# ShivangNagta/CS201_SAH-BVH_Ray_Tracer

Hardware: AMD Instinct MI355X
Metric: Mrays/s at 1080p, 10k spheres; 1/2/4/8 GPU + CPU baseline (higher is better)
Workload: dtype f32

## Files before the change

cs201_sah-bvh_ray_tracer_amd/abi.py:

```python
import ctypes as C

import numpy as np

VEC3 = ("<f4", (3,))

SPHERE = np.dtype([("center", *VEC3), ("radius", "<f4"), ("color", "u1", (4,))])
RAY = np.dtype([("origin", *VEC3), ("direction", *VEC3)])
AABB = np.dtype([("min", *VEC3), ("max", *VEC3)])
HIT = np.dtype([("t", "<f4"), ("point", *VEC3), ("normal", *VEC3),
                ("hit", "<i4"), ("sphere", "<i4"), ("pad", "<i4")])
NODE = np.dtype([("bmin", *VEC3), ("bmax", *VEC3), ("sphere", "<i4"), ("skip", "<u4")])
CAMERA = np.dtype([("position", *VEC3), ("forward", *VEC3), ("right", *VEC3), ("up", *VEC3),
                   ("yaw", "<f4"), ("pitch", "<f4"), ("fov", "<f4"), ("move", "<i4")])

NODE_EMPTY = 0x80000000
SKIP_MASK = 0x7FFFFFFF

GEO = np.dtype(("<f4", (4,)))
DNODE = np.dtype([("bmin", *VEC3), ("bmax", *VEC3), ("sphere", "<i4"), ("skip", "<u4"),
                  ("geo", "<f4", (4,)), ("pad", "<u4", (4,))])
PNODE = np.dtype([("c0", "<f4", (6,)), ("c1", "<f4", (6,)), ("ref0", "<u4"), ("ref1", "<u4"),
                  ("flat", "<u4"), ("end", "<u4")])
HSLOT = np.dtype([("box", "<u4", (3,)), ("ref", "<u4")])
HNODE = np.dtype([("slot", HSLOT, (4,))])
# ... 190 lines not shown
    ("mirt_accum_download", I, [P, P, C.c_size_t]),
    ("mirt_ctx_share_accum", I, [P, P]),
    ("mirt_ctx_share_scene", I, [P, P]),
    ("mirt_ctx_scene_id", C.c_uint64, [P]),
    ("mirt_trace_rays", I, [P, P, I, I, I, C.c_uint64, C.c_uint32, P]),
    ("mirt_trace_rays_at", I, [P, P, I, I, I, C.c_uint64, C.c_uint32, C.c_uint32, P]),
    ("mirt_camera_rays_uv", I, [P, P, I, I, P, I, P]),
    ("mirt_bvh_overlay", I, [P, P, I, I, I, P]),
    ("mirt_intersect_rays", I, [P, P, I, I, P]),
    ("mirt_any_hit_rays", I, [P, P, I, I, P]),
    ("mirt_sphere_pairs", I, [P, P, P, I, P]),
    ("mirt_aabb_pairs", I, [P, P, P, I, P]),
    ("mirt_hemisphere_probe", I, [P, P, P, P, P, I, P, P]),
    ("mirt_coop_geometry", I, [I, C.c_uint64, P, P, P, P]),
    ("mirt_pixel_rows", I, [I, I, I, I, I, I, P, C.c_int64, P]),
    ("mirt_exact_t_pairs", I, [C.c_int64, P, P, P, P, P, P, P, P]),
    ("mirt_sqrt_form_sweep", I, [P, P, P]),
    ("mirt_box_form_pairs", I, [P, P, P, P, I, I, P]),
    ("mirt_sphere_form_pairs", I, [P, P, P, P, I, I, P]),
    ("mirt_camera_rays", I, [P, P, P, P]),
    ("mirt_count_frame", I, [P, P, P, P]),
    ("mirt_wave_stats", I, [P, P, P, P, I]),
    ("mirt_ctx_stream", P, [P]),
    ("mirt_last_kernel_ms", C.c_float, [P]),
    ("mirt_last_phase_ms", I, [P, C.POINTER(C.c_float)]),
    ("mirt_phase_log", I, [P, C.POINTER(C.c_float), I]),
    ("mirt_bounce_stats", I, [P, P, P, P, I]),
    ("mirt_set_option", I, [P, I, I]),
    ("mirt_get_option", I, [P, I]),
    ("mirt_primary_cache_stats_get", I, [P, P]),
    ("mirt_primary_cache_read", I, [P, P, P, C.c_size_t]),
    ("mirt_primary_cache_write", I, [P, P, P, C.c_size_t]),
    ("mirt_dropin_init", I, [I, I, I]),
    ("mirt_dropin_release", None, []),
# ... 31 lines not shown

OPT_TRAVERSAL, OPT_FAST_SLAB, OPT_BLOCK_WAVES, OPT_DEFER, OPT_BOUNCE_THRESHOLD, OPT_PRUNE, OPT_ORDERED = (
    1, 2, 3, 4, 5, 6, 7)
OPT_BOUNCE_BLOCKS, OPT_QUAD_DRAIN, OPT_LEAF_BATCH, OPT_QUAD_BATCH, OPT_ZERO_COPY = 9, 11, 14, 15, 17
OPT_QUEUE_ORDER, OPT_DEBUG_STALL_MS = 18, 19
OPT_CONFIRM_ONCE, OPT_DEBUG_FAIL_CONFIRM = 21, 22
OPT_BUILD_FINISH = 23
OPT_PRIMARY_CACHE = 24
PCACHE_BYPASS, PCACHE_FILL, PCACHE_HIT = 0, 1, 2
PCACHE_KIND = {PCACHE_BYPASS: "bypass", PCACHE_FILL: "fill", PCACHE_HIT: "hit"}
PCACHE_REASON = {0: "", 1: "EMPTY", 2: "SCENE", 3: "CAMERA", 4: "GEOMETRY", 5: "OFF", 6: "SCHEDULE", 7: "JITTER",
                 8: "PLANES"}
BOUNCE_STATS_WORDS = 23
TRAV_TILE, TRAV_WAVEFRONT = 0, 5
BOX_FORM_SLAB, BOX_FORM_SLAB_BOX, BOX_FORM_CONS, BOX_FORM_CONS_BOUNCE, BOX_FORM_CONS_CAMERA = 0, 1, 2, 3, 4
MULTI_COPY, MULTI_HOST_DIRECT, MULTI_QUEUE_AHEAD = 1, 2, 4
MULTI_FULL_GRID = 1
MULTI_OPT_TIMEOUT_MS, MULTI_OPT_EMULATE_WORLD, MULTI_OPT_EMULATE_RANK, MULTI_OPT_DIRECT_COPY = 256, 257, 258, 259
MULTI_OPT_COPY_STREAM = 260
MULTI_OPT_GATHER_SELF, MULTI_OPT_LEAD_SKIP = 261, 262
```

cs201_sah-bvh_ray_tracer_amd/csrc/coop.h:

```cpp
#pragma once
#include <cstdint>

#include "rng.h"
#include "shard.h"

namespace mirt {

MIRT_HD uint32_t coop_group_shift(uint32_t np)
{
    const uint32_t ceil_log2 = np <= 1u ? 0u : 32u - (uint32_t)__builtin_clz(np - 1u);
    return 6u - ceil_log2;
}
MIRT_HD uint32_t coop_lane_rank(uint32_t lane, uint32_t shift) { return lane >> shift; }
MIRT_HD uint32_t coop_lane_try(uint32_t lane, uint32_t shift) { return lane & ((1u << shift) - 1u); }

MIRT_HD int coop_first_accept(uint64_t accepted, uint32_t rank, uint32_t shift)
{
    uint64_t bits = accepted >> ((rank << shift) & 63u);
    if (shift < 6u) bits &= (1ull << (1u << shift)) - 1ull;
    return bits ? __builtin_ctzll(bits) : -1;
}

struct MagicDiv {
    uint32_t mul, shift;
// ... 17 lines not shown
};
inline RowMagic row_magic_make(int width, int shard_rows, int row_block)
{
    return RowMagic{magic_div_make((uint32_t)width), magic_div_make((uint32_t)shard_rows),
                    magic_div_make((uint32_t)row_block)};
}

MIRT_HD int magic_row_to_y(const RowMagic& m, int r, int samples, int shard_rows, int row_block, int shard,
                           int num_shards, int lead_skip)
{
    if (samples > 1) r -= (int)magic_div((uint32_t)r, (uint32_t)shard_rows, m.shard_rows) * shard_rows;
    const int blk = (int)magic_div((uint32_t)r, (uint32_t)row_block, m.row_block);
    return shard_block(shard, blk, num_shards, lead_skip) * row_block + (r - blk * row_block);
}

}
```

cs201_sah-bvh_ray_tracer_amd/csrc/coop_host.cpp:

```cpp
#include "coop.h"
#include "internal.h"

using namespace mirt;

extern "C" int mirt_coop_geometry(int num_pending, uint64_t accepted, int32_t* group, int32_t* lane_rank,
                                  int32_t* lane_try, int32_t* first_accept)
{
    if (num_pending < 1 || num_pending > 64 || !group || !lane_rank || !lane_try || !first_accept) {
        set_error("mirt_coop_geometry: invalid arguments");
        return MIRT_E_INVALID;
    }
    const uint32_t shift = coop_group_shift((uint32_t)num_pending);
    *group = (int32_t)(1u << shift);
    for (uint32_t i = 0; i < 64; i++) {
        lane_rank[i] = (int32_t)coop_lane_rank(i, shift);
        lane_try[i] = (int32_t)coop_lane_try(i, shift);
    }
    for (uint32_t r = 0; r < (uint32_t)num_pending; r++) first_accept[r] = coop_first_accept(accepted, r, shift);
    return MIRT_OK;
}

extern "C" int mirt_pixel_rows(int width, int shard_rows, int samples, int row_block, int shard, int num_shards,
                               const uint32_t* pixels, int64_t n, int32_t* out)
{
// ... 1 lines not shown
        shard >= num_shards || n < 0 || (n > 0 && (!pixels || !out))) {
        set_error("mirt_pixel_rows: invalid arguments");
        return MIRT_E_INVALID;
    }
    const RowMagic m = row_magic_make(width, shard_rows, row_block);
    for (int64_t i = 0; i < n; i++) {
        const uint32_t p = pixels[i];
        const uint32_t r = magic_div(p, (uint32_t)width, m.width);
        out[4 * i] = (int32_t)r;
        out[4 * i + 1] = (int32_t)(p - r * (uint32_t)width);
        out[4 * i + 2] = magic_row_to_y(m, (int)r, samples, shard_rows, row_block, shard, num_shards, 0);
        out[4 * i + 3] = (int32_t)magic_div(r, (uint32_t)shard_rows, m.shard_rows);
    }
    return MIRT_OK;
}
```

cs201_sah-bvh_ray_tracer_amd/csrc/render.hip:

```cpp
#include <hip/hip_runtime.h>

#include <cmath>
#include <cstdint>
#include <algorithm>
#include <map>
#include <mutex>
#include <cstring>
#include <new>
#include <type_traits>
#include <vector>

#include "coop.h"
#include "internal.h"
#include "shard.h"
#include "trace.h"

using namespace mirt;

namespace {

struct FrameConst {
    float px, py, pz;
    float fx, fy, fz;
    float hx, hy, hz;
// ... 399 lines not shown
        return;
    }
    if (pm) {
        const int leader = __builtin_ctzll(pm);
        uint32_t base = 0;
        if (lane == leader) base = atomicAdd(&qctl[0], (uint32_t)__popcll(pm));
        base = __builtin_amdgcn_readlane(base, leader);
        if (push) queue[base + lanes_below(pm)] = rec;
    }
}

constexpr bool kBoundedSlab = true;
__device__ __forceinline__ SlabRay bounce_slab_ray(const DevScene& sc, const Ray& ray)
{
    SlabRay s = slab_ray(ray);
    s.generic = s.generic ||
                !(sc.o_bound > 0.0f && fmaxf(fabsf(ray.ox), fmaxf(fabsf(ray.oy), fabsf(ray.oz))) <= sc.o_bound);
    return s;
}

__host__ __device__ inline bool origin_within_4c(float o_bound, float o_inf)
{
    return o_bound > 0.0f && o_inf <= 4.0f * o_bound;
}

template <int WALK>
struct BounceWalk;
template <>
struct BounceWalk<0> {
    DfsWalk w;
    __device__ void start(const DevScene& sc) { w = DfsWalk{0u, sc.num_nodes}; }
    __device__ void stop() { w = DfsWalk{kPNone, 0u}; }
// ... 6 lines not shown
        if (w.cur >= w.end) w.cur = kPNone;
    }
};
template <int WALK>
struct WideBounceWalk {
    WideWalk w;
    lds_uint4* hc = nullptr;
    uint32_t hc_n = 0;
    __device__ void start(const DevScene& sc) { w = wide_walk_start(sc, true); }
    __device__ void stop() { w = WideWalk{kPNone, 0u, 0u}; }
    __device__ bool walking() const { return wide_walking(w); }
    template <bool FAST, bool GD = false, bool DEFER = false>
    __device__ void step(const DevScene& sc, const SlabRay& sr, const SphRay& sp, Prune& pr, uint32_t* stk,
                         float& bt, int& bs, Counters& cnt, GateDiag* gd = nullptr, int* lvl = nullptr)
    {
        wide_lane_step<FAST, false, WALK == 4, kBoundedSlab && WALK != 4, GD, DEFER>(sc, sr, sp, pr, w, stk, bt, bs,
                                                                                     cnt, hc, hc_n, gd, lvl);
    }
};
template <>
struct BounceWalk<2> : WideBounceWalk<2> {};
template <>
struct BounceWalk<4> : WideBounceWalk<4> {};


inline size_t bounce_lds_bytes(int depth) { return sizeof(uint32_t) * 256 * (size_t)std::max(depth - 1, 1); }

__device__ __forceinline__ uint64_t chain_key(const FrameConst& f, uint32_t pixel)
{
    const int r = (int)magic_div(pixel, (uint32_t)f.width, f.magic.width), x = (int)(pixel - (uint32_t)r * (uint32_t)f.width);
    return pixel_key(f.seed, (uint32_t)(shard_row_to_y(f, r) * f.width + x), row_sample(f, r));
}

__device__ __forceinline__ bool shade_level(const DevScene& sc, const FrameConst& f, Ray& ray, float best_t,
                                            int best_s, int& level, uint32_t& k, uint64_t key, uint32_t* cs,
                                            int cstride, uint32_t base0, uint32_t pixel, uint32_t* __restrict__ out,
                                            float* __restrict__ acc, bool store)
{
    uint32_t tail = 255u << 24;
    int stored = level - 1;
    if (best_s < 0) {
// ... 49 lines not shown
    for (;;) {
        while (solo_step<FAST, kWideStack * 64, BND>(sc, sr, sp, pr, w, wst, best_t, best_s, hc, hc_n, lane)) {
        }
        if (!shade_level(sc, f, ray, best_t, best_s, level, k, chain_key(f, pixel), cs, kWideStride, base0, pixel, out,
                         acc, lane == 0))
            return;
        sr = bounce_slab_ray(sc, ray);
        sp = sph_ray(ray);
        w = SoloWalk{lane < 4 ? sc.wide_root : kPNone, 0u, 0u};
        best_t = INFINITY;
        best_s = -1;
        pr = prune_off();
    }
}

#define MIRT_BOUNCE_ATTR __attribute__((amdgpu_waves_per_eu(MIRT_BOUNCE_WAVES)))
template <bool FAST, int WALK, bool DIAG = false>
__global__ __launch_bounds__(256) MIRT_BOUNCE_ATTR void bounce_kernel(DevScene sc, FrameConst f, uint32_t* __restrict__ out,
                                                     float* __restrict__ acc, const BounceRec* __restrict__ queue,
                                                     uint32_t* __restrict__ qctl, int threshold, int quad_drain,
                                                     int lvl_mode, int fail_n,
                                                     uint64_t* __restrict__ diag = nullptr)
{
    uint64_t dg_it = 0, dg_lanes = 0, dg_it_x = 0, dg_lanes_x = 0, dg_tx = 0, dg_qit = 0, dg_tq = 0;
    const uint64_t dg_t0 = DIAG ? __builtin_amdgcn_s_memrealtime() : 0;
    uint32_t dg_steps = 0, dg_chain = 0, dg_walk_max = 0, dg_chain_max = 0;
    uint64_t dg_seg = 0, dg_fb = 0, dg_it_gate = 0, dg_it_t = 0, dg_it_box = 0;
    uint32_t dg_conf = 0, dg_conf_fail = 0, dg_fb_exact = 0;
    GateDiag gd{0, 0, 0, 0, 0, false, false, false};
    constexpr bool LANE4 = WALK == 2 || WALK == 4;
// ... 1 lines not shown
    constexpr int cstride = 256;
    extern __shared__ uint32_t cstack[];
    __shared__ uint32_t wstack[LANE4 ? kWideStack * kWideStride : 1];
    __shared__ uint32_t qsrc[LANE4 ? 4 * 16 : 1];
    __shared__ uint4 hcache[LANE4 ? 4 * kHCache : 1];
    uint32_t hc_n = 0;
    if constexpr (LANE4) {
        hc_n = min((uint32_t)kHCache, sc.num_hnodes);
        const uint4* src = (const uint4*)sc.hnodes;
        for (uint32_t i = threadIdx.x; i < 4 * hc_n; i += blockDim.x) hcache[i] = src[i];
        __syncthreads();
    }
    uint32_t tid4 = threadIdx.x << 2;
    if (DEFER) asm volatile("" : "+v"(tid4));
    const uint32_t tid = DEFER ? tid4 >> 2 : threadIdx.x;
    uint32_t* cs = DEFER ? (uint32_t*)((char*)cstack + tid4) : cstack + threadIdx.x;
    uint32_t* stk = DEFER ? (uint32_t*)((char*)wstack + tid4) : wstack + (LANE4 ? threadIdx.x : 0);
    Counters cnt{0, 0, 0, 0, 0};
    const uint32_t n = __builtin_amdgcn_readfirstlane(qctl[0]);
    uint32_t seg = blockIdx.x % kQSeg, segs_left = kQSeg;
    bool has = false, exhausted = false;
    Ray ray{0, 0, 0, 0, 0, 0};
    SlabRay sr = bounce_slab_ray(sc, ray);
    SphRay sp = sph_ray(ray);
    Prune pr = prune_off();
    BounceWalk<WALK> w;
    if constexpr (LANE4) {
        w.hc = (lds_uint4*)hcache;
        w.hc_n = hc_n;
    }
    w.stop();
    uint32_t pixel = 0, k = 0, base0 = 0;
    int level = 0, best_s = -1;
    float best_t = INFINITY;
    for (;;) {
        const uint64_t need = __ballot(!has);
        while (need && !exhausted) {
            const int leader = __builtin_ctzll(need);
            const uint32_t lo = (uint32_t)((uint64_t)n * seg / kQSeg);
            const uint32_t sz = (uint32_t)((uint64_t)n * (seg + 1) / kQSeg) - lo;
            uint32_t b = 0;
            if ((tid & 63) == leader) b = atomicAdd(&qctl[kQLine * (1 + seg)], (uint32_t)__popcll(need));
            b = __builtin_amdgcn_readlane(b, leader);
            if (b + (uint32_t)__popcll(need) >= sz) {
                seg = seg + 1 == kQSeg ? 0 : seg + 1;
                if (--segs_left == 0) exhausted = true;
            }
            if (!has) {
                const uint32_t lane0 = tid & 63;
                const uint32_t idx = b + (uint32_t)__popcll(need & ((1ull << lane0) - 1));
                if (idx < sz) {
                    const BounceRec rec = queue[lo + idx];
                    ray = Ray{rec.ox, rec.oy, rec.oz, rec.dx, rec.dy, rec.dz};
                    sr = bounce_slab_ray(sc, ray);
                    sp = sph_ray(ray);
                    pixel = rec.pixel;
                    k = rec.k;
                    base0 = rec.base0;
                    level = DEFER ? 1 | lvl_mode : 1;
                    w.start(sc);
                    best_t = INFINITY;
                    best_s = -1;
                    pr = prune_off();
                    has = true;
                }
            }
            if (b < sz) break;
        }
        if (!__ballot(has)) break;
        if (DIAG && exhausted && !dg_tx) dg_tx = __builtin_amdgcn_s_memrealtime();
        auto to_drain = [&]() {
            uint32_t busy = (uint32_t)__popcll(__ballot(has));
            asm volatile("" : "+s"(busy));
// ... 34 lines not shown
                dg_it_box += __ballot(gd.st_box) ? 1u : 0u;
            } else if constexpr (DEFER) {
                if (has && w.walking())
                    w.template step<FAST, false, true>(sc, sr, sp, pr, stk, best_t, best_s, cnt, nullptr, &level);
            } else {
                if (has && w.walking()) w.template step<FAST>(sc, sr, sp, pr, stk, best_t, best_s, cnt);
            }
        }
        if constexpr (DEFER) {
            const bool handover = to_drain();
            if (has && (handover || !w.walking()) && !(level & kExactWalk) && best_s >= 0) {
                best_s = confirm_leaf(sc, sr, best_s);
                if (fail_n) {
                    uint32_t fn = (uint32_t)fail_n;
                    asm volatile("" : "+s"(fn));
                    if (pixel % fn == 0) best_s = -1;
                }
                if (DIAG) {
                    dg_conf++;
                    dg_conf_fail += best_s < 0 ? 1u : 0u;
                }
                if (best_s < 0) {
                    level |= kExactWalk;
                    w.start(sc);
                    best_t = INFINITY;
                    pr = prune_off();
                }
            }
            if (handover) break;
        }
        bool go = false;
        float nn[3] = {0.0f, 0.0f, 0.0f};
        uint64_t key = 0;
        if constexpr (WALK == 4) {
            if (has && !w.walking()) {
                go = shade_level(sc, f, ray, best_t, best_s, level, k, chain_key(f, pixel), cs, cstride, base0, pixel,
                                 out, acc, true);
                has = go;
            }
        } else if (has && !w.walking()) {
            if (DEFER) level &= ~kExactWalk;
            if (DIAG) {
                dg_walk_max = max(dg_walk_max, dg_steps);
                dg_chain += dg_steps;
                dg_steps = 0;
            }
            uint32_t tail = 255u << 24;
            int stored = level - 1;
            if (best_s < 0) {
                tail = sky_rgba(ray.dy);
            } else {
                cs[(level - 1) * cstride] = sc.color[best_s];
                stored = level;
                if (level + 1 < f.depth) {
                    float p[3];
                    hit_point_normal(ray, best_t, sc.geo[best_s], p, nn);
                    ray.ox = p[0];
                    ray.oy = p[1];
                    ray.oz = p[2];
                    key = chain_key(f, pixel);
                    level++;
                    go = true;
                }
            }
            if (!go) {
                uint32_t c = tail;
                for (int l = stored - 1; l >= 0; l--) c = blend_rgba(cs[l * cstride], c);
                store_pixel(f, out, acc, pixel, blend_rgba(base0, c));
                has = false;
                if (DIAG) {
                    dg_chain_max = max(dg_chain_max, dg_chain);
                    dg_chain = 0;
                }
            }
        }
        if (WALK != 4 && __ballot(go)) hemisphere_wave(key, k, nn, go, ray.dx, ray.dy, ray.dz, tid & 63);
        if (go) {
            sr = bounce_slab_ray(sc, ray);
            sp = sph_ray(ray);
            w.start(sc);
            best_t = INFINITY;
            best_s = -1;
            pr = prune_off();
            if (DEFER) level |= lvl_mode;
        }
    }
    if constexpr (DEFER) level &= ~kExactWalk;
    if constexpr (LANE4) {
        const uint64_t busy = __ballot(has);
        if (busy) {
            const uint32_t lane = tid & 63, wv = tid >> 6;
            if (has) qsrc[wv * 16 + lanes_below(busy)] = lane;
            __builtin_amdgcn_fence(__ATOMIC_RELEASE, "wavefront");
            __builtin_amdgcn_wave_barrier();
            __builtin_amdgcn_fence(__ATOMIC_ACQUIRE, "wavefront");
            const uint32_t q = lane >> 2;
            const bool qhas = q < (uint32_t)__popcll(busy);
            const uint32_t src = qsrc[wv * 16 + (qhas ? q : 0)];
            auto pull = [&](uint32_t v) { return (uint32_t)__builtin_amdgcn_ds_bpermute((int)(src << 2), (int)v); };
            auto pullf = [&](float v) { return __uint_as_float(pull(__float_as_uint(v))); };
            ray = Ray{pullf(ray.ox), pullf(ray.oy), pullf(ray.oz), pullf(ray.dx), pullf(ray.dy), pullf(ray.dz)};
            pixel = pull(pixel);
            k = pull(k);
            level = (int)pull((uint32_t)level);
            base0 = pull(base0);
            best_t = pullf(best_t);
            best_s = (int)pull((uint32_t)best_s);
            pr = Prune{pullf(pr.m), pullf(pr.lim)};
            const WideWalk& lw = w.w;
            QuadWalk qw{pull(lw.cur), pull(lw.end), pull(lw.top)};
            has = qhas;
            if (!qhas) qw.cur = kPNone;
            sr = bounce_slab_ray(sc, ray);
            sp = sph_ray(ray);
            uint32_t* qstk = wstack + (tid & ~63u) + src;
            uint32_t* qcs = cstack + (tid & ~63u) + src;
            if (DIAG) dg_tq = __builtin_amdgcn_s_memrealtime();
            while (__ballot(has)) {
                if (DIAG) dg_qit++;
                if (!DIAG) {
                    const uint64_t rays = __ballot(has && (lane & 3) == 0);
                    if (__popcll(rays) == 1) {
                        solo_chain<FAST, kBoundedSlab && WALK != 4>(sc, f, __builtin_ctzll(rays), ray, best_t, best_s, pr,
                                                                    qw, level, k, pixel,
                                         base0, src, wstack + (tid & ~63u), cstack + (tid & ~63u),
                                         out, acc, (lds_uint4*)hcache, hc_n, lane);
                        break;
                    }
                }
                if (has && qw.cur != kPNone)
                    quad_step<FAST, kWideStride, kWideStack, kBoundedSlab && WALK != 4>(sc, sr, sp, pr, qw, qstk, best_t,
                                                                                        best_s,
                                                             (lds_uint4*)hcache, hc_n, lane);
                if (has && qw.cur == kPNone) {
                    if (shade_level(sc, f, ray, best_t, best_s, level, k, chain_key(f, pixel), qcs, kWideStride, base0, pixel, out,
                                    acc, (lane & 3) == 0)) {
                        sr = bounce_slab_ray(sc, ray);
                        sp = sph_ray(ray);
                        qw = QuadWalk{sc.wide_root, 0u, 0u};
                        best_t = INFINITY;
// ... 301 lines not shown
        nd.g = make_float4(0.0f, 0.0f, 0.0f, 0.0f);
        pass = slab<true>(sr, pr, nd);
        break;
    }
    case MIRT_BOX_FORM_SLAB_BOX:
        pass = slab_box<true>(sr, pr, b.min.x, b.min.y, b.min.z, b.max.x, b.max.y, b.max.z, near);
        break;
    case MIRT_BOX_FORM_CONS:
        pass = slab_cons<false>(sr, pr, b.min.x, b.min.y, b.min.z, b.max.x, b.max.y, b.max.z, near);
        break;
    case MIRT_BOX_FORM_CONS_BOUNCE:
        sr = bounce_slab_ray(sc, ray);
        pass = slab_cons<true>(sr, pr, b.min.x, b.min.y, b.min.z, b.max.x, b.max.y, b.max.z, near);
        break;
    default:
        sr.generic = sr.generic ||
                     !origin_within_4c(sc.o_bound, fmaxf(fabsf(ray.ox), fmaxf(fabsf(ray.oy), fabsf(ray.oz))));
        pass = slab_cons<true>(sr, pr, b.min.x, b.min.y, b.min.z, b.max.x, b.max.y, b.max.z, near);
        break;
    }
    out[i] = pass ? 1 : 0;
}

template <int MODE>
__global__ void sphere_form_pairs_kernel(const mirt_ray* __restrict__ rays, const mirt_sphere* __restrict__ sph,
                                         const float* __restrict__ best, int n, uint32_t* __restrict__ out)
{
    const int i = blockIdx.x * blockDim.x + threadIdx.x;
    if (i >= n) return;
    const mirt_ray rr = rays[i];
    const Ray ray{rr.origin.x, rr.origin.y, rr.origin.z, rr.direction.x, rr.direction.y, rr.direction.z};
    const float4 g = make_float4(sph[i].center.x, sph[i].center.y, sph[i].center.z, sph[i].radius);
    if constexpr (MODE == 3) {
        bool f64 = false;
        (void)sphere_t<true>(sph_ray(ray), g, best[i], &f64);
        out[i] = f64 ? 1u : 0u;
// ... 1840 lines not shown
    if (n == 0) return MIRT_OK;
    const size_t rb = sizeof(mirt_ray) * (size_t)n, bb = sizeof(mirt_aabb) * (size_t)n, fb = 4 * (size_t)n;
    int rc = ensure(&c->d_in, &c->in_cap, rb + bb + fb + 16);
    if (!rc) rc = ensure(&c->d_res, &c->res_cap, 4 * (size_t)n);
    if (rc) return rc;
    char* din = (char*)c->d_in;
    HIP_TRY(hipMemcpyAsync(din, rays, rb, hipMemcpyHostToDevice, c->stream));
    HIP_TRY(hipMemcpyAsync(din + rb, boxes, bb, hipMemcpyHostToDevice, c->stream));
    HIP_TRY(hipMemcpyAsync(din + rb + bb, best, fb, hipMemcpyHostToDevice, c->stream));
    box_form_pairs_kernel<<<(n + 255) / 256, 256, 0, c->stream>>>(dev_scene(c), (const mirt_ray*)din,
                                                                 (const mirt_aabb*)(din + rb),
                                                                 (const float*)(din + rb + bb), n, form,
                                                                 (int32_t*)c->d_res);
    HIP_TRY(hipGetLastError());
    HIP_TRY(hipMemcpyAsync(out, c->d_res, 4 * (size_t)n, hipMemcpyDeviceToHost, c->stream));
    HIP_TRY(hipStreamSynchronize(c->stream));
    return MIRT_OK;
}

int mirt_sphere_form_pairs(mirt_ctx* c, const mirt_ray* rays, const mirt_sphere* spheres, const float* best, int n,
                           int fast, uint32_t* out)
{
    if (!ctx_ok(c, false, "mirt_sphere_form_pairs")) return MIRT_E_INVALID;
    if (n < 0 || fast < 0 || fast > 3 || (n > 0 && (!rays || !spheres || !best || !out))) {
        set_error("mirt_sphere_form_pairs: invalid arguments");
        return MIRT_E_INVALID;
    }
    if (n == 0) return MIRT_OK;
    const size_t rb = sizeof(mirt_ray) * (size_t)n, sb = sizeof(mirt_sphere) * (size_t)n, fb = 4 * (size_t)n;
    int rc = ensure(&c->d_in, &c->in_cap, rb + sb + fb + 16);
// ... 255 lines not shown
```

cs201_sah-bvh_ray_tracer_amd/csrc/trace.h:

```cpp
#pragma once
#include <hip/hip_runtime.h>

#include <cstdint>

#include "../../include/mirt.h"
#include "coop.h"
#include "exact_t.h"
#include "layout.h"
#include "rng.h"

namespace mirt {

constexpr float kEps = 0.000001f;
constexpr int kMaxDepth = 8;

struct DevScene {
    const DNode* nodes;
    const mirt_node* nodes32;
    const float4* geo;
    const uint32_t* color;
    uint32_t num_nodes;
    int num_spheres;
    int prune;
    float r_max;
// ... 93 lines not shown
        x = y = z = 0.0f;
    }
}

__device__ __forceinline__ float dot3(float ax, float ay, float az, float bx, float by, float bz)
{
    float s = ax * bx;
    s = s + ay * by;
    return s + az * bz;
}

struct SlabRay {
    float ox, oy, oz, dx, dy, dz;
    float ix, iy, iz;
    bool zx, zy, zz;
    bool generic;
};

__device__ __forceinline__ SlabRay slab_ray(const Ray& r)
{
    SlabRay s;
    s.ox = r.ox;
    s.oy = r.oy;
    s.oz = r.oz;
    s.dx = r.dx;
    s.dy = r.dy;
    s.dz = r.dz;
    s.zx = r.dx == 0.0f;
    s.zy = r.dy == 0.0f;
    s.zz = r.dz == 0.0f;
    const float tiny = 0x1p-40f;
    s.generic = !(fabsf(r.dx) >= tiny && fabsf(r.dy) >= tiny && fabsf(r.dz) >= tiny);
    s.ix = 1.0f / r.dx;
    s.iy = 1.0f / r.dy;
    s.iz = 1.0f / r.dz;
    return s;
}

__device__ __forceinline__ bool slab_test(const SlabRay& r, float x0, float y0, float z0, float x1, float y1,
                                          float z1)
{
    float tx1 = -INFINITY, tx2 = INFINITY, ty1 = -INFINITY, ty2 = INFINITY, tz1 = -INFINITY, tz2 = INFINITY;
    if (!r.zx) {
        tx1 = (x0 - r.ox) / r.dx;
        tx2 = (x1 - r.ox) / r.dx;
    }
    if (!r.zy) {
        ty1 = (y0 - r.oy) / r.dy;
        ty2 = (y1 - r.oy) / r.dy;
    }
// ... 510 lines not shown

__device__ __forceinline__ void cx(float& ka, uint32_t& ra, float& kb, uint32_t& rb)
{
    const bool sw = kb < ka;
    const float k = sw ? kb : ka;
    const uint32_t r = sw ? rb : ra;
    kb = sw ? ka : kb;
    rb = sw ? ra : rb;
    ka = k;
    ra = r;
}

__device__ __forceinline__ float h_lo(uint32_t v) { return (float)__builtin_bit_cast(_Float16, (uint16_t)(v & 0xffffu)); }
__device__ __forceinline__ float h_hi(uint32_t v) { return (float)__builtin_bit_cast(_Float16, (uint16_t)(v >> 16)); }

struct GateDiag {
    uint32_t gates, gates_t, gates_box, lanes_t, lanes_box;
    bool st_gate, st_t, st_box;
    __device__ __forceinline__ void gate(bool et, bool eb)
    {
        const uint64_t act = __ballot(true);
        const bool lead =
            __builtin_amdgcn_mbcnt_hi((uint32_t)(act >> 32), __builtin_amdgcn_mbcnt_lo((uint32_t)act, 0u)) == 0;
        const bool any_t = __ballot(et) != 0, any_box = __ballot(eb) != 0;
        gates += lead ? 1u : 0u;
        gates_t += (lead && any_t) ? 1u : 0u;
        gates_box += (lead && any_box) ? 1u : 0u;
        lanes_t += et ? 1u : 0u;
        lanes_box += eb ? 1u : 0u;
        st_gate = true;
// ... 77 lines not shown
{
    const float t = sphere_t<true>(sp, g, best_t);
    if (t > 0.0f) {
        const float4* lp = (const float4*)(sc.leaf_box + (ref & ~kPLeaf));
        const float4 l0 = lp[0], l1 = lp[1];
        const int si = __float_as_int(l1.z);
        float e;
        if ((t < best_t || si > best_s) && slab_box<true>(sr, pr, l0.x, l0.y, l0.z, l0.w, l1.x, l1.y, e)) {
            best_t = t;
            best_s = si;
            if (sc.prune) prune_update(pr, sc, sr.ox, sr.oy, sr.oz, sp.a4(), t);
        }
    }
}

template <bool FAST, bool COUNT, bool BATCH = false, bool BND = false, bool GD = false, bool DEFER = false>
__device__ __forceinline__ void wide_lane_step(const DevScene& sc, const SlabRay& sr, const SphRay& sp, Prune& pr,
                                               WideWalk& w, uint32_t* stk, float& best_t, int& best_s, Counters& cnt,
                                               lds_uint4* hc = nullptr, uint32_t hc_n = 0, GateDiag* gd = nullptr,
                                               int* lvl = nullptr)
{
    static_assert(!DEFER || (FAST && !COUNT && !BATCH), "the deferred gates are the timed lane loop's");
    if (COUNT) cnt.steps++;
    if (w.end) {
        lane_step<FAST, COUNT, true>(sc, sr, sp, pr, w.cur, best_t, best_s, cnt);
        if (w.cur >= w.end) {
            w.end = 0;
            wide_walk_pop(w, stk);
        }
        return;
    }
// ... 3 lines not shown
    {
        uint4 s0, s1, s2, s3;
        if (w.cur < hc_n) {
            lds_uint4* p = hc + 4 * w.cur;
            s0 = lds_load(p);
            s1 = lds_load(p + 1);
            s2 = lds_load(p + 2);
            s3 = lds_load(p + 3);
        } else {
            const uint4* p = (const uint4*)(sc.hnodes + w.cur);
            s0 = p[0];
            s1 = p[1];
            s2 = p[2];
            s3 = p[3];
        }
        auto test = [&](const uint4& q, float& e) {
            if (COUNT && q.w != kPNone) cnt.nodes++;
            const bool pass =
                slab_cons<BND>(sr, pr, h_lo(q.x), h_lo(q.y), h_lo(q.z), h_hi(q.x), h_hi(q.y), h_hi(q.z), e);
            return pass & (q.w != kPNone);
        };
        h0 = test(s0, e0);
        h1 = test(s1, e1);
        h2 = test(s2, e2);
        h3 = test(s3, e3);
        q3 = make_uint4(s0.w, s1.w, s2.w, s3.w);
    }
    uint32_t lm = (uint32_t)(h0 && (q3.x & kPLeaf)) | (uint32_t)(h1 && (q3.y & kPLeaf)) << 1 |
                  (uint32_t)(h2 && (q3.z & kPLeaf)) << 2 | (uint32_t)(h3 && (q3.w & kPLeaf)) << 3;
    h0 = h0 && !(lm & 1);
    h1 = h1 && !(lm & 2);
    h2 = h2 && !(lm & 4);
    h3 = h3 && !(lm & 8);
    const uint32_t n = (uint32_t)h0 + (uint32_t)h1 + (uint32_t)h2 + (uint32_t)h3;
// ... 648 lines not shown
```

cs201_sah-bvh_ray_tracer_amd/renderer.py:

```python
import ctypes as C
import os

import numpy as np

from . import abi
from .lib import MirtError, check, load

ptr = abi.ptr


class RandState:

    def __init__(self, seed=1):
        self.st = abi.RandState()
        load().mirt_srand(C.byref(self.st), seed)

    def rand(self):
        return load().mirt_rand(C.byref(self.st))


def create_random_spheres(n, seed=1, state=None):
    st = state or RandState(seed)
    out = np.zeros(n, abi.SPHERE)
    check(load().mirt_scene_random(C.byref(st.st), ptr(out), n), "mirt_scene_random")
# ... 569 lines not shown
        boxes = np.ascontiguousarray(boxes, abi.AABB)
        out = np.zeros(len(rays), np.int32)
        check(self.L.mirt_aabb_pairs(self.h, ptr(rays), ptr(boxes), len(rays), ptr(out)), "mirt_aabb_pairs")
        return out

    def box_form_pairs(self, rays, boxes, best, form):
        rays = np.ascontiguousarray(rays, abi.RAY)
        boxes = np.ascontiguousarray(boxes, abi.AABB)
        best = np.ascontiguousarray(best, np.float32)
        assert len(boxes) == len(rays) and len(best) == len(rays)
        out = np.zeros(len(rays), np.int32)
        check(self.L.mirt_box_form_pairs(self.h, ptr(rays), ptr(boxes), ptr(best), len(rays), form, ptr(out)),
              "mirt_box_form_pairs")
        return out

    def sphere_form_pairs(self, rays, spheres, best, fast=True):
        rays = np.ascontiguousarray(rays, abi.RAY)
        spheres = np.ascontiguousarray(spheres, abi.SPHERE)
        best = np.ascontiguousarray(best, np.float32)
        assert len(spheres) == len(rays) and len(best) == len(rays)
        out = np.zeros(len(rays), np.uint32)
        check(self.L.mirt_sphere_form_pairs(self.h, ptr(rays), ptr(spheres), ptr(best), len(rays), int(fast),
                                            ptr(out)), "mirt_sphere_form_pairs")
        return out.view(np.float32)

    def sqrt_form_sweep(self):
        bad, first = C.c_uint64(), C.c_uint32()
        check(self.L.mirt_sqrt_form_sweep(self.h, C.byref(bad), C.byref(first)), "mirt_sqrt_form_sweep")
        return bad.value, first.value

# ... 190 lines not shown
```

include/mirt.h:

```cpp
#ifndef MIRT_H
#define MIRT_H

#include <stddef.h>
#include <stdint.h>

#ifdef __cplusplus
extern "C" {
#endif


typedef struct mirt_vec3 { float x, y, z; } mirt_vec3;
typedef struct mirt_rgba8 { uint8_t r, g, b, a; } mirt_rgba8;
typedef struct mirt_sphere {
    mirt_vec3 center;
    float radius;
    mirt_rgba8 color;
} mirt_sphere;
typedef struct mirt_ray { mirt_vec3 origin, direction; } mirt_ray;
typedef struct mirt_camera {
    mirt_vec3 position, forward, right, up;
    float yaw, pitch, fov;
    int move;
} mirt_camera;
typedef struct mirt_aabb { mirt_vec3 min, max; } mirt_aabb;
// ... 225 lines not shown

int mirt_intersect_rays(mirt_ctx *ctx, const mirt_ray *rays, int n, int use_bvh, mirt_hit *out);

int mirt_any_hit_rays(mirt_ctx *ctx, const mirt_ray *rays, int n, int use_bvh, int32_t *out);

int mirt_sphere_pairs(mirt_ctx *ctx, const mirt_ray *rays, const mirt_sphere *spheres, int n, mirt_hit *out);
int mirt_aabb_pairs(mirt_ctx *ctx, const mirt_ray *rays, const mirt_aabb *boxes, int n, int32_t *out);

int mirt_hemisphere_probe(mirt_ctx *ctx, const uint64_t *keys, const uint32_t *k0, const float *normals,
                          const int32_t *need, int n, float *out_dir, uint32_t *out_k);

int mirt_coop_geometry(int num_pending, uint64_t accepted, int32_t *group, int32_t *lane_rank, int32_t *lane_try,
                       int32_t *first_accept);
int mirt_pixel_rows(int width, int shard_rows, int samples, int row_block, int shard, int num_shards,
                    const uint32_t *pixels, int64_t n, int32_t *out);

enum { MIRT_BOX_FORM_SLAB = 0,
       MIRT_BOX_FORM_SLAB_BOX = 1,
       MIRT_BOX_FORM_CONS = 2,
       MIRT_BOX_FORM_CONS_BOUNCE = 3,
       MIRT_BOX_FORM_CONS_CAMERA = 4   };
int mirt_box_form_pairs(mirt_ctx *ctx, const mirt_ray *rays, const mirt_aabb *boxes, const float *best, int n,
                        int form, int32_t *out);
int mirt_sphere_form_pairs(mirt_ctx *ctx, const mirt_ray *rays, const mirt_sphere *spheres, const float *best,
                           int n, int fast, uint32_t *out);
int mirt_exact_t_pairs(int64_t n, const float *b, const float *disc, const float *d2a, const float *s,
                       const float *rs, const float *rd, float *th, uint8_t *certified);
int mirt_sqrt_form_sweep(mirt_ctx *ctx, uint64_t *mismatches, uint32_t *first);
int mirt_build_partition_probe(mirt_ctx *ctx, const float *centre, int n, const int32_t *seg, int nseg,
                               const float *split, int32_t *perm);
typedef struct mirt_scene_layout_info {
    int32_t  encloses, ordered, leaf_big;
    float    r_max, c_max, o_bound;
    uint32_t num_pnodes, num_hnodes, num_leaves, wide_root;
    uint64_t leaf_box_off;
} mirt_scene_layout_info;
enum { MIRT_LAYOUT_DNODES = 0, MIRT_LAYOUT_GEO = 1, MIRT_LAYOUT_COLOR = 2, MIRT_LAYOUT_PNODES = 3,
       MIRT_LAYOUT_HNODES = 4, MIRT_LAYOUT_HAUX = 5, MIRT_LAYOUT_LEAF_GEO = 6, MIRT_LAYOUT_LEAF_BOX = 7,
       MIRT_LAYOUT_NDEPTH = 8 };
int64_t mirt_scene_layout(const mirt_sphere *spheres, int num_spheres, const mirt_node *nodes, int num_nodes,
// ... 63 lines not shown
```

Before: 2998.

## Park cold bounce chain state in LDS and add octant-swapped fp16 slab tests

Moves the per-lane pixel, k and base0 chain values out of registers into three new LDS rows ahead of the colour stack, reading and writing them only where they are needed. Adds a precomputed ray octant word so the wide BVH slab test can swap the fp16 min/max planes with alignbit, removing per-axis min/max selection, with a fallback for generic rays. The aims are lower register pressure in the bounce kernel and a cheaper box test, at the cost of extra LDS traffic and footprint and a more complex test path. New host test entry points expose the layout and the slot test form.

```diff
diff --git a/cs201_sah-bvh_ray_tracer_amd/abi.py b/cs201_sah-bvh_ray_tracer_amd/abi.py
--- a/cs201_sah-bvh_ray_tracer_amd/abi.py
+++ b/cs201_sah-bvh_ray_tracer_amd/abi.py
@@ -228,10 +228,12 @@
     ("mirt_hemisphere_probe", I, [P, P, P, P, P, I, P, P]),
     ("mirt_coop_geometry", I, [I, C.c_uint64, P, P, P, P]),
     ("mirt_pixel_rows", I, [I, I, I, I, I, I, P, C.c_int64, P]),
+    ("mirt_bounce_lds_layout", I, [I, I, P, P, P, P]),
     ("mirt_exact_t_pairs", I, [C.c_int64, P, P, P, P, P, P, P, P]),
     ("mirt_sqrt_form_sweep", I, [P, P, P]),
     ("mirt_box_form_pairs", I, [P, P, P, P, I, I, P]),
     ("mirt_sphere_form_pairs", I, [P, P, P, P, I, I, P]),
+    ("mirt_slot_form_pairs", I, [P, P, P, P, I, I, P, P]),
     ("mirt_camera_rays", I, [P, P, P, P]),
     ("mirt_count_frame", I, [P, P, P, P]),
     ("mirt_wave_stats", I, [P, P, P, P, I]),
@@ -293,6 +295,7 @@
 BOUNCE_STATS_WORDS = 23
 TRAV_TILE, TRAV_WAVEFRONT = 0, 5
 BOX_FORM_SLAB, BOX_FORM_SLAB_BOX, BOX_FORM_CONS, BOX_FORM_CONS_BOUNCE, BOX_FORM_CONS_CAMERA = 0, 1, 2, 3, 4
+SLOT_FORM_OCTANT, SLOT_FORM_BOUNCE = 1, 2
 MULTI_COPY, MULTI_HOST_DIRECT, MULTI_QUEUE_AHEAD = 1, 2, 4
 MULTI_FULL_GRID = 1
 MULTI_OPT_TIMEOUT_MS, MULTI_OPT_EMULATE_WORLD, MULTI_OPT_EMULATE_RANK, MULTI_OPT_DIRECT_COPY = 256, 257, 258, 259
diff --git a/cs201_sah-bvh_ray_tracer_amd/csrc/coop.h b/cs201_sah-bvh_ray_tracer_amd/csrc/coop.h
--- a/cs201_sah-bvh_ray_tracer_amd/csrc/coop.h
+++ b/cs201_sah-bvh_ray_tracer_amd/csrc/coop.h
@@ -55,4 +55,11 @@
     return shard_block(shard, blk, num_shards, lead_skip) * row_block + (r - blk * row_block);
 }
 
+constexpr uint32_t kBounceCols = 256;
+enum : uint32_t { kParkPixel = 0, kParkBase0 = 1, kParkK = 2, kParkRows = 3 };
+MIRT_HD uint32_t bounce_colour_rows(int depth) { return depth > 2 ? (uint32_t)depth - 1u : 1u; }
+MIRT_HD uint32_t park_word(uint32_t row, uint32_t col) { return row * kBounceCols + col; }
+MIRT_HD uint32_t colour_word(uint32_t level_row, uint32_t col) { return (kParkRows + level_row) * kBounceCols + col; }
+MIRT_HD uint32_t bounce_lds_words(int depth) { return (kParkRows + bounce_colour_rows(depth)) * kBounceCols; }
+
 }
diff --git a/cs201_sah-bvh_ray_tracer_amd/csrc/coop_host.cpp b/cs201_sah-bvh_ray_tracer_amd/csrc/coop_host.cpp
--- a/cs201_sah-bvh_ray_tracer_amd/csrc/coop_host.cpp
+++ b/cs201_sah-bvh_ray_tracer_amd/csrc/coop_host.cpp
@@ -39,3 +39,21 @@
     }
     return MIRT_OK;
 }
+
+extern "C" int mirt_bounce_lds_layout(int depth, int column, int32_t* park, int32_t* colour, int32_t* colour_rows,
+                                      int64_t* bytes)
+{
+    if (depth < 0 || depth > 8 || column < 0 || column >= (int)kBounceCols || !park || !colour || !colour_rows ||
+        !bytes) {
+        set_error("mirt_bounce_lds_layout: invalid arguments");
+        return MIRT_E_INVALID;
+    }
+    const uint32_t rows = bounce_colour_rows(depth);
+    park[0] = (int32_t)park_word(kParkPixel, (uint32_t)column);
+    park[1] = (int32_t)park_word(kParkBase0, (uint32_t)column);
+    park[2] = (int32_t)park_word(kParkK, (uint32_t)column);
+    for (uint32_t r = 0; r < rows; r++) colour[r] = (int32_t)colour_word(r, (uint32_t)column);
+    *colour_rows = (int32_t)rows;
+    *bytes = (int64_t)sizeof(uint32_t) * bounce_lds_words(depth);
+    return MIRT_OK;
+}
diff --git a/cs201_sah-bvh_ray_tracer_amd/csrc/render.hip b/cs201_sah-bvh_ray_tracer_amd/csrc/render.hip
--- a/cs201_sah-bvh_ray_tracer_amd/csrc/render.hip
+++ b/cs201_sah-bvh_ray_tracer_amd/csrc/render.hip
@@ -437,8 +437,8 @@
 __device__ __forceinline__ SlabRay bounce_slab_ray(const DevScene& sc, const Ray& ray)
 {
     SlabRay s = slab_ray(ray);
-    s.generic = s.generic ||
-                !(sc.o_bound > 0.0f && fmaxf(fabsf(ray.ox), fmaxf(fabsf(ray.oy), fabsf(ray.oz))) <= sc.o_bound);
+    slab_set_generic(s, s.generic || !(sc.o_bound > 0.0f &&
+                                       fmaxf(fabsf(ray.ox), fmaxf(fabsf(ray.oy), fabsf(ray.oz))) <= sc.o_bound));
     return s;
 }
 
@@ -475,8 +475,8 @@
     __device__ void step(const DevScene& sc, const SlabRay& sr, const SphRay& sp, Prune& pr, uint32_t* stk,
                          float& bt, int& bs, Counters& cnt, GateDiag* gd = nullptr, int* lvl = nullptr)
     {
-        wide_lane_step<FAST, false, WALK == 4, kBoundedSlab && WALK != 4, GD, DEFER>(sc, sr, sp, pr, w, stk, bt, bs,
-                                                                                     cnt, hc, hc_n, gd, lvl);
+        wide_lane_step<FAST, false, WALK == 4, kBoundedSlab && WALK != 4, GD, DEFER, kOctantSlots && WALK != 4>(
+            sc, sr, sp, pr, w, stk, bt, bs, cnt, hc, hc_n, gd, lvl);
     }
 };
 template <>
@@ -485,7 +485,7 @@
 struct BounceWalk<4> : WideBounceWalk<4> {};
 
 
-inline size_t bounce_lds_bytes(int depth) { return sizeof(uint32_t) * 256 * (size_t)std::max(depth - 1, 1); }
+inline size_t bounce_lds_bytes(int depth) { return sizeof(uint32_t) * (size_t)bounce_lds_words(depth); }
 
 __device__ __forceinline__ uint64_t chain_key(const FrameConst& f, uint32_t pixel)
 {
@@ -565,6 +565,12 @@
     }
 }
 
+struct ChainCold {
+    uint32_t* col;
+    __device__ __forceinline__ uint32_t get(uint32_t row) const { return col[park_word(row, 0)]; }
+    __device__ __forceinline__ void set(uint32_t row, uint32_t v) { col[park_word(row, 0)] = v; }
+};
+
 #define MIRT_BOUNCE_ATTR __attribute__((amdgpu_waves_per_eu(MIRT_BOUNCE_WAVES)))
 template <bool FAST, int WALK, bool DIAG = false>
 __global__ __launch_bounds__(256) MIRT_BOUNCE_ATTR void bounce_kernel(DevScene sc, FrameConst f, uint32_t* __restrict__ out,
@@ -596,7 +602,8 @@
     uint32_t tid4 = threadIdx.x << 2;
     if (DEFER) asm volatile("" : "+v"(tid4));
     const uint32_t tid = DEFER ? tid4 >> 2 : threadIdx.x;
-    uint32_t* cs = DEFER ? (uint32_t*)((char*)cstack + tid4) : cstack + threadIdx.x;
+    ChainCold cold{DEFER ? (uint32_t*)((char*)cstack + tid4) : cstack + threadIdx.x};
+    uint32_t* cs = cold.col + colour_word(0, 0);
     uint32_t* stk = DEFER ? (uint32_t*)((char*)wstack + tid4) : wstack + (LANE4 ? threadIdx.x : 0);
     Counters cnt{0, 0, 0, 0, 0};
     const uint32_t n = __builtin_amdgcn_readfirstlane(qctl[0]);
@@ -612,7 +619,6 @@
         w.hc_n = hc_n;
     }
     w.stop();
-    uint32_t pixel = 0, k = 0, base0 = 0;
     int level = 0, best_s = -1;
     float best_t = INFINITY;
     for (;;) {
@@ -636,9 +642,9 @@
                     ray = Ray{rec.ox, rec.oy, rec.oz, rec.dx, rec.dy, rec.dz};
                     sr = bounce_slab_ray(sc, ray);
                     sp = sph_ray(ray);
-                    pixel = rec.pixel;
-                    k = rec.k;
-                    base0 = rec.base0;
+                    cold.set(kParkPixel, rec.pixel);
+                    cold.set(kParkK, rec.k);
+                    cold.set(kParkBase0, rec.base0);
                     level = DEFER ? 1 | lvl_mode : 1;
                     w.start(sc);
                     best_t = INFINITY;
@@ -703,7 +709,7 @@
                 if (fail_n) {
                     uint32_t fn = (uint32_t)fail_n;
                     asm volatile("" : "+s"(fn));
-                    if (pixel % fn == 0) best_s = -1;
+                    if (cold.get(kParkPixel) % fn == 0) best_s = -1;
                 }
                 if (DIAG) {
                     dg_conf++;
@@ -723,8 +729,11 @@
         uint64_t key = 0;
         if constexpr (WALK == 4) {
             if (has && !w.walking()) {
-                go = shade_level(sc, f, ray, best_t, best_s, level, k, chain_key(f, pixel), cs, cstride, base0, pixel,
-                                 out, acc, true);
+                const uint32_t pixel = cold.get(kParkPixel);
+                uint32_t k = cold.get(kParkK);
+                go = shade_level(sc, f, ray, best_t, best_s, level, k, chain_key(f, pixel), cs, cstride,
+                                 cold.get(kParkBase0), pixel, out, acc, true);
+                cold.set(kParkK, k);
                 has = go;
             }
         } else if (has && !w.walking()) {
@@ -747,7 +756,7 @@
                     ray.ox = p[0];
                     ray.oy = p[1];
                     ray.oz = p[2];
-                    key = chain_key(f, pixel);
+                    key = chain_key(f, cold.get(kParkPixel));
                     level++;
                     go = true;
                 }
@@ -755,7 +764,7 @@
             if (!go) {
                 uint32_t c = tail;
                 for (int l = stored - 1; l >= 0; l--) c = blend_rgba(cs[l * cstride], c);
-                store_pixel(f, out, acc, pixel, blend_rgba(base0, c));
+                store_pixel(f, out, acc, cold.get(kParkPixel), blend_rgba(cold.get(kParkBase0), c));
                 has = false;
                 if (DIAG) {
                     dg_chain_max = max(dg_chain_max, dg_chain);
@@ -763,7 +772,11 @@
                 }
             }
         }
-        if (WALK != 4 && __ballot(go)) hemisphere_wave(key, k, nn, go, ray.dx, ray.dy, ray.dz, tid & 63);
+        if (WALK != 4 && __ballot(go)) {
+            uint32_t k = go ? cold.get(kParkK) : 0u;
+            hemisphere_wave(key, k, nn, go, ray.dx, ray.dy, ray.dz, tid & 63);
+            if (go) cold.set(kParkK, k);
+        }
         if (go) {
             sr = bounce_slab_ray(sc, ray);
             sp = sph_ray(ray);
@@ -789,10 +802,7 @@
             auto pull = [&](uint32_t v) { return (uint32_t)__builtin_amdgcn_ds_bpermute((int)(src << 2), (int)v); };
             auto pullf = [&](float v) { return __uint_as_float(pull(__float_as_uint(v))); };
             ray = Ray{pullf(ray.ox), pullf(ray.oy), pullf(ray.oz), pullf(ray.dx), pullf(ray.dy), pullf(ray.dz)};
-            pixel = pull(pixel);
-            k = pull(k);
             level = (int)pull((uint32_t)level);
-            base0 = pull(base0);
             best_t = pullf(best_t);
             best_s = (int)pull((uint32_t)best_s);
             pr = Prune{pullf(pr.m), pullf(pr.lim)};
@@ -803,7 +813,10 @@
             sr = bounce_slab_ray(sc, ray);
             sp = sph_ray(ray);
             uint32_t* qstk = wstack + (tid & ~63u) + src;
-            uint32_t* qcs = cstack + (tid & ~63u) + src;
+            uint32_t* qcs = cstack + colour_word(0, (tid & ~63u) + src);
+            const ChainCold qcold{cstack + (tid & ~63u) + src};
+            const uint32_t pixel = qcold.get(kParkPixel), base0 = qcold.get(kParkBase0);
+            uint32_t k = qcold.get(kParkK);
             if (DIAG) dg_tq = __builtin_amdgcn_s_memrealtime();
             while (__ballot(has)) {
                 if (DIAG) dg_qit++;
@@ -812,7 +825,7 @@
                     if (__popcll(rays) == 1) {
                         solo_chain<FAST, kBoundedSlab && WALK != 4>(sc, f, __builtin_ctzll(rays), ray, best_t, best_s, pr,
                                                                     qw, level, k, pixel,
-                                         base0, src, wstack + (tid & ~63u), cstack + (tid & ~63u),
+                                         base0, src, wstack + (tid & ~63u), cstack + colour_word(0, tid & ~63u),
                                          out, acc, (lds_uint4*)hcache, hc_n, lane);
                         break;
                     }
@@ -1144,12 +1157,41 @@
         pass = slab_cons<true>(sr, pr, b.min.x, b.min.y, b.min.z, b.max.x, b.max.y, b.max.z, near);
         break;
     default:
-        sr.generic = sr.generic ||
-                     !origin_within_4c(sc.o_bound, fmaxf(fabsf(ray.ox), fmaxf(fabsf(ray.oy), fabsf(ray.oz))));
+        slab_set_generic(sr, sr.generic || !origin_within_4c(sc.o_bound, fmaxf(fabsf(ray.ox),
+                                                                                  fmaxf(fabsf(ray.oy), fabsf(ray.oz)))));
         pass = slab_cons<true>(sr, pr, b.min.x, b.min.y, b.min.z, b.max.x, b.max.y, b.max.z, near);
         break;
     }
     out[i] = pass ? 1 : 0;
+}
+
+__global__ void slot_form_pairs_kernel(DevScene sc, const mirt_ray* __restrict__ rays,
+                                       const mirt_aabb* __restrict__ boxes, const float* __restrict__ best, int n,
+                                       int form, uint32_t* __restrict__ out)
+{
+    const int i = blockIdx.x * blockDim.x + threadIdx.x;
+    if (i >= n) return;
+    const mirt_ray rr = rays[i];
+    const Ray ray{rr.origin.x, rr.origin.y, rr.origin.z, rr.direction.x, rr.direction.y, rr.direction.z};
+    const mirt_aabb b = boxes[i];
+    const float bt = best[i];
+    Prune pr = prune_start(sc, ray.ox, ray.oy, ray.oz);
+    if (sc.prune && bt < INFINITY) prune_update(pr, sc, ray.ox, ray.oy, ray.oz, sph_ray(ray).a4(), bt);
+    auto half = [](float v) { return (uint32_t)__builtin_bit_cast(uint16_t, (_Float16)v); };
+    const uint32_t qx = half(b.min.x) | half(b.max.x) << 16, qy = half(b.min.y) | half(b.max.y) << 16,
+                   qz = half(b.min.z) | half(b.max.z) << 16;
+    const SlabRay sr = (form & MIRT_SLOT_FORM_BOUNCE) ? bounce_slab_ray(sc, ray) : slab_ray(ray);
+    const OctAmt amt = oct_amounts(sr);
+    float near = 0.0f;
+    bool pass;
+    switch (form) {
+    case 0: pass = slab_cons_slot<false, false>(sr, amt, pr, qx, qy, qz, near); break;
+    case MIRT_SLOT_FORM_OCTANT: pass = slab_cons_slot<false, true>(sr, amt, pr, qx, qy, qz, near); break;
+    case MIRT_SLOT_FORM_BOUNCE: pass = slab_cons_slot<true, false>(sr, amt, pr, qx, qy, qz, near); break;
+    default: pass = slab_cons_slot<true, true>(sr, amt, pr, qx, qy, qz, near); break;
+    }
+    out[i] = pass ? 1u : 0u;
+    out[(size_t)n + i] = __float_as_uint(near);
 }
 
 template <int MODE>
@@ -3020,6 +3062,43 @@
                                                                  (int32_t*)c->d_res);
     HIP_TRY(hipGetLastError());
     HIP_TRY(hipMemcpyAsync(out, c->d_res, 4 * (size_t)n, hipMemcpyDeviceToHost, c->stream));
+    HIP_TRY(hipStreamSynchronize(c->stream));
+    return MIRT_OK;
+}
+
+int mirt_slot_form_pairs(mirt_ctx* c, const mirt_ray* rays, const mirt_aabb* boxes, const float* best, int n, int form,
+                         int32_t* out_pass, uint32_t* out_near)
+{
+    if (!ctx_ok(c, true, "mirt_slot_form_pairs")) return MIRT_E_NOSCENE;
+    if (n < 0 || form < 0 || form > (MIRT_SLOT_FORM_OCTANT | MIRT_SLOT_FORM_BOUNCE) ||
+        (n > 0 && (!rays || !boxes || !best || !out_pass || !out_near))) {
+        set_error("mirt_slot_form_pairs: invalid arguments");
+        return MIRT_E_INVALID;
+    }
+    for (int i = 0; i < n; i++) {
+        const float v[6] = {boxes[i].min.x, boxes[i].min.y, boxes[i].min.z, boxes[i].max.x, boxes[i].max.y, boxes[i].max.z};
+        for (int k = 0; k < 6; k++)
+            if (!((float)(_Float16)v[k] == v[k]) || !(v[k % 3] <= v[k % 3 + 3])) {
+                set_error("mirt_slot_form_pairs: box %d is not a slot's (fp16 planes, lo <= hi)", i);
+                return MIRT_E_INVALID;
+            }
+    }
+    if (n == 0) return MIRT_OK;
+    const size_t rb = sizeof(mirt_ray) * (size_t)n, bb = sizeof(mirt_aabb) * (size_t)n, fb = 4 * (size_t)n;
+    int rc = ensure(&c->d_in, &c->in_cap, rb + bb + fb + 16);
+    if (!rc) rc = ensure(&c->d_res, &c->res_cap, 2 * fb);
+    if (rc) return rc;
+    char* din = (char*)c->d_in;
+    HIP_TRY(hipMemcpyAsync(din, rays, rb, hipMemcpyHostToDevice, c->stream));
+    HIP_TRY(hipMemcpyAsync(din + rb, boxes, bb, hipMemcpyHostToDevice, c->stream));
+    HIP_TRY(hipMemcpyAsync(din + rb + bb, best, fb, hipMemcpyHostToDevice, c->stream));
+    slot_form_pairs_kernel<<<(n + 255) / 256, 256, 0, c->stream>>>(dev_scene(c), (const mirt_ray*)din,
+                                                                  (const mirt_aabb*)(din + rb),
+                                                                  (const float*)(din + rb + bb), n, form,
+                                                                  (uint32_t*)c->d_res);
+    HIP_TRY(hipGetLastError());
+    HIP_TRY(hipMemcpyAsync(out_pass, c->d_res, fb, hipMemcpyDeviceToHost, c->stream));
+    HIP_TRY(hipMemcpyAsync(out_near, (char*)c->d_res + fb, fb, hipMemcpyDeviceToHost, c->stream));
     HIP_TRY(hipStreamSynchronize(c->stream));
     return MIRT_OK;
 }
diff --git a/cs201_sah-bvh_ray_tracer_amd/csrc/trace.h b/cs201_sah-bvh_ray_tracer_amd/csrc/trace.h
--- a/cs201_sah-bvh_ray_tracer_amd/csrc/trace.h
+++ b/cs201_sah-bvh_ray_tracer_amd/csrc/trace.h
@@ -131,8 +131,16 @@
     float ox, oy, oz, dx, dy, dz;
     float ix, iy, iz;
     bool zx, zy, zz;
+    uint32_t oct;
     bool generic;
 };
+constexpr uint32_t kOctGeneric = 1u << 24;
+
+__device__ __forceinline__ void slab_set_generic(SlabRay& s, bool g)
+{
+    s.generic = g;
+    s.oct = (s.oct & ~kOctGeneric) | (g ? kOctGeneric : 0u);
+}
 
 __device__ __forceinline__ SlabRay slab_ray(const Ray& r)
 {
@@ -151,6 +159,8 @@
     s.ix = 1.0f / r.dx;
     s.iy = 1.0f / r.dy;
     s.iz = 1.0f / r.dz;
+    s.oct = (__float_as_uint(s.ix) >> 31) << 4 | (__float_as_uint(s.iy) >> 31) << 12 |
+            (__float_as_uint(s.iz) >> 31) << 20 | (s.generic ? kOctGeneric : 0u);
     return s;
 }
 
@@ -691,6 +701,59 @@
 __device__ __forceinline__ float h_lo(uint32_t v) { return (float)__builtin_bit_cast(_Float16, (uint16_t)(v & 0xffffu)); }
 __device__ __forceinline__ float h_hi(uint32_t v) { return (float)__builtin_bit_cast(_Float16, (uint16_t)(v >> 16)); }
 
+struct OctAmt {
+    uint32_t x, y, z;
+};
+__device__ __forceinline__ OctAmt oct_amounts(const SlabRay& r)
+{
+    return {r.oct, r.oct >> 8, r.oct >> 16};
+}
+
+template <bool BND, bool OCT>
+__device__ __forceinline__ bool slab_cons_slot(const SlabRay& r, const OctAmt& amt, const Prune& p, uint32_t qx,
+                                               uint32_t qy, uint32_t qz, float& near)
+{
+    if constexpr (!OCT) {
+        return slab_cons<BND>(r, p, h_lo(qx), h_lo(qy), h_lo(qz), h_hi(qx), h_hi(qy), h_hi(qz), near);
+    } else {
+        const uint32_t rx = __builtin_amdgcn_alignbit(qx, qx, amt.x);
+        const uint32_t ry = __builtin_amdgcn_alignbit(qy, qy, amt.y);
+        const uint32_t rz = __builtin_amdgcn_alignbit(qz, qz, amt.z);
+        const float oix = r.ox * r.ix, oiy = r.oy * r.iy, oiz = r.oz * r.iz;
+        const float mo = fmaxf(fabsf(oix), fmaxf(fabsf(oiy), fabsf(oiz))) * 0x1p-22f;
+        const float nx = fmaf(h_lo(rx), r.ix, -oix), fx = fmaf(h_hi(rx), r.ix, -oix);
+        const float ny = fmaf(h_lo(ry), r.iy, -oiy), fy = fmaf(h_hi(ry), r.iy, -oiy);
+        const float nz = fmaf(h_lo(rz), r.iz, -oiz), fz = fmaf(h_hi(rz), r.iz, -oiz);
+        const float tmin = fmaxf(nx, fmaxf(ny, nz));
+        const float tmax = fminf(fx, fminf(fy, fz));
+        near = tmin;
+        bool pass;
+        if (BND) {
+            const float ent =
+                fmaxf(fmaf(-p.m, fabsf(r.ix), nx), fmaxf(fmaf(-p.m, fabsf(r.iy), ny), fmaf(-p.m, fabsf(r.iz), nz)));
+            pass = !(ent > p.lim) & !(tmax < fmaxf(tmin, kEps));
+        } else {
+            constexpr float c = 1.0f - 0x1p-20f;
+            const float entry =
+                fmaxf(fmaf(nx, c, -fmaf(p.m, fabsf(r.ix), mo)),
+                      fmaxf(fmaf(ny, c, -fmaf(p.m, fabsf(r.iy), mo)), fmaf(nz, c, -fmaf(p.m, fabsf(r.iz), mo))));
+            const float m = fmaf(fabsf(tmin) + fabsf(tmax), 0x1p-20f, 2.0f * mo);
+            pass = !(entry > p.lim) & !(tmax + m < fmaxf(tmin, kEps));
+        }
+        if (r.oct & kOctGeneric) {
+            near = 0.0f;
+            const float x0 = h_lo(qx), y0 = h_lo(qy), z0 = h_lo(qz), x1 = h_hi(qx), y1 = h_hi(qy), z1 = h_hi(qz);
+            pass = !pruned_any(r, p, x0, y0, z0, x1, y1, z1) && slab_test(r, x0, y0, z0, x1, y1, z1);
+        }
+        return pass;
+    }
+}
+
+#ifndef MIRT_OCTANT_SLOTS
+#define MIRT_OCTANT_SLOTS 1
+#endif
+constexpr bool kOctantSlots = MIRT_OCTANT_SLOTS != 0;
+
 struct GateDiag {
     uint32_t gates, gates_t, gates_box, lanes_t, lanes_box;
     bool st_gate, st_t, st_box;
@@ -798,7 +861,8 @@
     }
 }
 
-template <bool FAST, bool COUNT, bool BATCH = false, bool BND = false, bool GD = false, bool DEFER = false>
+template <bool FAST, bool COUNT, bool BATCH = false, bool BND = false, bool GD = false, bool DEFER = false,
+          bool OCT = false>
 __device__ __forceinline__ void wide_lane_step(const DevScene& sc, const SlabRay& sr, const SphRay& sp, Prune& pr,
                                                WideWalk& w, uint32_t* stk, float& best_t, int& best_s, Counters& cnt,
                                                lds_uint4* hc = nullptr, uint32_t hc_n = 0, GateDiag* gd = nullptr,
@@ -832,10 +896,10 @@
             s2 = p[2];
             s3 = p[3];
         }
+        const OctAmt amt = OCT ? oct_amounts(sr) : OctAmt{0u, 0u, 0u};
         auto test = [&](const uint4& q, float& e) {
             if (COUNT && q.w != kPNone) cnt.nodes++;
-            const bool pass =
-                slab_cons<BND>(sr, pr, h_lo(q.x), h_lo(q.y), h_lo(q.z), h_hi(q.x), h_hi(q.y), h_hi(q.z), e);
+            const bool pass = slab_cons_slot<BND, OCT>(sr, amt, pr, q.x, q.y, q.z, e);
             return pass & (q.w != kPNone);
         };
         h0 = test(s0, e0);
diff --git a/cs201_sah-bvh_ray_tracer_amd/renderer.py b/cs201_sah-bvh_ray_tracer_amd/renderer.py
--- a/cs201_sah-bvh_ray_tracer_amd/renderer.py
+++ b/cs201_sah-bvh_ray_tracer_amd/renderer.py
@@ -607,6 +607,17 @@
               "mirt_box_form_pairs")
         return out
 
+    def slot_form_pairs(self, rays, boxes, best, form):
+        rays = np.ascontiguousarray(rays, abi.RAY)
+        boxes = np.ascontiguousarray(boxes, abi.AABB)
+        best = np.ascontiguousarray(best, np.float32)
+        assert len(boxes) == len(rays) and len(best) == len(rays)
+        out = np.zeros(len(rays), np.int32)
+        near = np.zeros(len(rays), np.uint32)
+        check(self.L.mirt_slot_form_pairs(self.h, ptr(rays), ptr(boxes), ptr(best), len(rays), form, ptr(out),
+                                          ptr(near)), "mirt_slot_form_pairs")
+        return out, near
+
     def sphere_form_pairs(self, rays, spheres, best, fast=True):
         rays = np.ascontiguousarray(rays, abi.RAY)
         spheres = np.ascontiguousarray(spheres, abi.SPHERE)
diff --git a/include/mirt.h b/include/mirt.h
--- a/include/mirt.h
+++ b/include/mirt.h
@@ -263,6 +263,8 @@
                        int32_t *first_accept);
 int mirt_pixel_rows(int width, int shard_rows, int samples, int row_block, int shard, int num_shards,
                     const uint32_t *pixels, int64_t n, int32_t *out);
+int mirt_bounce_lds_layout(int depth, int column, int32_t *park, int32_t *colour, int32_t *colour_rows,
+                           int64_t *bytes);
 
 enum { MIRT_BOX_FORM_SLAB = 0,
        MIRT_BOX_FORM_SLAB_BOX = 1,
@@ -273,6 +275,9 @@
                         int form, int32_t *out);
 int mirt_sphere_form_pairs(mirt_ctx *ctx, const mirt_ray *rays, const mirt_sphere *spheres, const float *best,
                            int n, int fast, uint32_t *out);
+enum { MIRT_SLOT_FORM_OCTANT = 1, MIRT_SLOT_FORM_BOUNCE = 2 };
+int mirt_slot_form_pairs(mirt_ctx *ctx, const mirt_ray *rays, const mirt_aabb *boxes, const float *best, int n,
+                         int form, int32_t *out_pass, uint32_t *out_near);
 int mirt_exact_t_pairs(int64_t n, const float *b, const float *disc, const float *d2a, const float *s,
                        const float *rs, const float *rd, float *th, uint8_t *certified);
 int mirt_sqrt_form_sweep(mirt_ctx *ctx, uint64_t *mismatches, uint32_t *first);
```

Result: no change. 2997 (median of 2 runs) (-0.0%).
